# ydwu4/dgl-hack

Measured on AMD Instinct MI355X. Metric: edges/sec + achieved HBM GB/s, GCN copy_u_sum on 100M-edge graph, 1/2/4/8 MI355X, higher is better.
Workload: dtype f32; 1 GPU; M1 copy_u_sum: RMAT scale 23, 100000000 edges, feat 64, int32 in-CSR; nodes=8388608, edges=100000000, feat=64, parallelism=single

## Files before the change

dgl-hack_amd/csrc/capi.cpp:

```cpp
#include <hip/hip_runtime.h>

#include <algorithm>
#include <cmath>
#include <atomic>
#include <cstdio>
#include <cstdlib>
#include <cstring>
#include <stdexcept>
#include <string>
#include <vector>

#include "internal.h"

using namespace dglmi;

namespace {

thread_local std::string g_last_error;

struct Error : std::runtime_error {
  using std::runtime_error::runtime_error;
};

#define DGLMI_CHECK(cond, msg)                                                     \
// ... 308 lines not shown
    prev = dst;
  }
}

void run_fast(const ReduceWalk& rw, int kind, int red, const float* x, const int32_t* x_map,
              const float* w, const int32_t* w_map, float* out, int64_t F, int64_t head_dim,
              hipStream_t s, const DGLMIEpilogue* epi, const float* xr) {
  const DGLMICsr& walk = rw.csr;
  if (rw.num_blocks > 1 && !rw.wide && red == RED_SUM && x_map == nullptr && walk.nnz > 0 &&
      kind == FAST_COPY_COL && rw.blocks != nullptr) {
    run_fast_blocked(rw, kind, x, w, w_map, out, F, head_dim, s, epi);
    return;
  }
  if (walk.nnz == 0) {
    launch_fill(out, walk.num_rows * F, identity_of(red), s);
    if (epi) launch_epilogue(out, walk.num_rows, F, epi->row_mul, epi->row_div, epi->bias, epi->addend, s);
    return;
  }
  FastArgs a;
  std::memset(&a, 0, sizeof(a));
  a.indptr = rw.idx(walk.indptr);
  a.rows = walk.rows;
  a.indices = walk.indices;
  a.eids = rw.idx(rw.eid_positions ? nullptr : walk.data);
  a.nnz = walk.nnz;
  a.num_rows = walk.num_rows;
  a.x = x;
  a.w = w;
  a.x_map = x_map;
  a.w_map = w_map;
  a.out = out;
  a.F = F;
  a.head_dim = head_dim;
  a.chunk = fast_chunk_edges(walk.nnz, F);
  a.xr = xr;
  if (kind == FAST_COPY_COL && red == RED_SUM && x_map == nullptr && fast_marked_supported(F) &&
      rw.marked != nullptr &&
      walk.num_cols * F * static_cast<int64_t>(sizeof(float)) >= kMarkedMinTableBytes) {
    a.indices = rw.marked;
    a.marked = 1;
    a.num_cols = walk.num_cols;
  }
  if (epi) {
    a.row_mul = epi->row_mul;
    a.row_div = epi->row_div;
    a.bias = epi->bias;
    a.addend = epi->addend;
  }
  if (kind == FAST_COL_MUL_EDGE_BCAST && !a.eids && head_dim == F && w_map == nullptr &&
      red == RED_SUM)
    kind = FAST_COL_MUL_POS;
  const DGLMIHubPlan* plan = rw.plan;
  if (plan != nullptr && !(kind == FAST_COPY_COL && red == RED_SUM && x_map == nullptr && epi == nullptr &&
                           !rw.wide && fast_marked_supported(F) && plan->num_hubs > 0))
    plan = nullptr;
  const int64_t virt = plan ? plan->num_blocks * plan->num_hubs : 0;
  Scratch part(no_workspace(), virt * F * static_cast<int64_t>(sizeof(float)), s);
  if (plan != nullptr) {
    DGLMI_CHECK(plan->nnz == walk.nnz && plan->hub_nnz <= walk.nnz && plan->num_blocks >= 1 &&
                    plan->rows && plan->indices && plan->indptr && plan->hub_rows,
                "hub plan does not belong to this CSR");
    a.indptr = IdxPtr{plan->indptr, 0};
    a.rows = plan->rows;
    a.indices = plan->marked ? plan->marked : plan->indices;
    a.marked = plan->marked != nullptr;
    a.num_cols = walk.num_cols;
    a.num_rows = virt + walk.num_rows;
    a.part = static_cast<float*>(part.ptr);
    a.virt_rows = virt;
    a.hub_rows = plan->hub_rows;
    a.num_hubs = plan->num_hubs;
    a.hub_blocks = plan->num_blocks;
    a.hub_nnz = plan->hub_nnz;
  }
  const CarryLayout lay((walk.nnz + a.chunk - 1) / a.chunk, F);
  Scratch carry(rw.ws, lay.bytes, s);
  lay.point(a, carry.ptr);
  launch_fast_reduce(kind, red, a, s);
  check_hip(hipGetLastError(), "fast reduce launch");
}

std::atomic<int> g_sddmm_order{DGLMI_SDDMM_ORDER_AUTO};

SddmmArgs sddmm_items(const DGLMIGraph* g, const DGLMICsr& walk, bool edge_operand,
                      int64_t row_floats) {
  SddmmArgs e;
  std::memset(&e, 0, sizeof(e));
  e.nnz = walk.nnz;
  bool coo = g->coo_src != nullptr && g->coo_dst != nullptr;
  if (coo) {
    const int forced = g_sddmm_order.load(std::memory_order_relaxed);
    if (forced == DGLMI_SDDMM_ORDER_CSR) coo = false;
    else if (forced != DGLMI_SDDMM_ORDER_COO)
      coo = edge_operand || row_floats < 32 || walk.nnz < 64 * std::max<int64_t>(walk.num_rows, 1);
  }
  if (coo) {
    e.rows = g->coo_dst;
    e.cols = g->coo_src;
    e.eids = IdxPtr{nullptr, 0};
  } else {
    e.rows = walk.rows;
    e.cols = walk.indices;
    e.eids = idx(g, walk.data);
  }
  return e;
}

EdgeArgs base_args(const DGLMIGraph* g, const DGLMICsr& walk) {
  EdgeArgs a;
  std::memset(&a, 0, sizeof(a));
  a.indptr = idx(g, walk.indptr);
  a.indices = walk.indices;
  a.eids = idx(g, walk.data);
  a.rows = walk.rows;
  a.num_rows = walk.num_rows;
  a.nnz = walk.nnz;
  a.len = 1;
  return a;
}

struct ReduceShape {
  bool bc;
  Bcast binfo;
  int64_t D, len;
};

// ... 1976 lines not shown
```

dgl-hack_amd/csrc/internal.h:

```cpp
#pragma once

#include <hip/hip_runtime.h>

#include <cstdint>

#include "../../include/dglmi.h"

namespace dglmi {

enum Role : int { ROLE_ROW = 0, ROLE_COL = 1, ROLE_EDGE = 2, ROLE_NONE = 3 };
enum Red : int { RED_SUM = 0, RED_MAX = 1, RED_MIN = 2, RED_PROD = 3, RED_NONE = 4 };
enum Op : int { OP_ADD = 0, OP_SUB = 1, OP_MUL = 2, OP_DIV = 3, OP_DOT = 4, OP_USE_LHS = 5 };

constexpr int kMaxDim = DGLMI_MAX_NDIM;

struct IdxPtr {
  const void* p;
  int wide;
  __host__ __device__ __forceinline__ int64_t operator[](int64_t i) const {
    return wide ? static_cast<const int64_t*>(p)[i]
                : static_cast<int64_t>(static_cast<const int32_t*>(p)[i]);
  }
  __host__ __device__ __forceinline__ explicit operator bool() const { return p != nullptr; }
};
// ... 240 lines not shown
  int pack;
  float* stat_pk;
};
bool softmax_supported(int64_t H);

bool project_supported(int64_t K, int64_t N);
int project_instance(int64_t K, int64_t N);
void launch_project(const float* X, int64_t M, int64_t K, const float* W, int64_t swk, int64_t swn,
                    int64_t N, const float* bias, float* Y, hipStream_t s);
int64_t softmax_chunk_edges(int64_t nnz, int64_t H);
int64_t softmax_owned_carry_bytes(int64_t nnz, int64_t H);
void launch_edge_softmax(const SoftmaxArgs& a, bool backward, hipStream_t s);
void launch_sm_row_sums(const SoftmaxArgs& a, hipStream_t s);

enum FastKind : int {
  FAST_COPY_COL = 0,
  FAST_COPY_EDGE = 1,
  FAST_COL_MUL_EDGE = 2,
  FAST_COL_MUL_EDGE_BCAST = 3,
  FAST_COL_TIE = 4,
  FAST_COL_MUL_POS = 5,
};
struct FastArgs {
  IdxPtr indptr;
  const int32_t* rows;
  const int32_t* indices;
  IdxPtr eids;
  int64_t nnz;
  int64_t num_rows;
  const float* x;
  const float* w;
  const int32_t* x_map;
  const int32_t* w_map;
  float* out;
  int64_t F;
  int64_t head_dim;
  float* carry;
  int32_t* seg_cnt;
  int64_t chunk;
  const float* row_mul;
  const float* row_div;
  const float* bias;
  const float* addend;
  int marked;
  const float* xr;
  int64_t num_cols;
  float* part;
  int64_t virt_rows;
  const int32_t* hub_rows;
  int64_t num_hubs;
  int64_t hub_blocks;
  int64_t hub_nnz;
  int64_t plan_wgs;
};
int64_t fast_chunk_edges(int64_t nnz, int64_t F);
int64_t fast_workspace_bytes(int64_t nnz, int64_t F);
bool fast_supported(int kind, int64_t F, int64_t head_dim);
void launch_fast_reduce(int kind, int red, const FastArgs& a, hipStream_t s);
void launch_mark_cold(const int32_t* cols, int64_t nnz, IdxPtr deg_indptr, int32_t thresh,
                      int32_t* out_cols, hipStream_t s);
inline bool fast_marked_supported(int64_t F) { return F > 32 && F <= 256 && F % 4 == 0; }
constexpr int64_t kMarkedMinTableBytes = int64_t(256) << 20;

struct GatArgs {
  const int32_t* indptr;
  const int32_t* rows;
  const int32_t* indices;
  int64_t nnz;
  int64_t num_rows;
  int H, D;
  int64_t F;
  float slope;
  const float* ft;
  const float* el;
  const float* er;
  float* out;
  float* m;
  float* l;
  const float* go;
  const float* fo;
  const float* m_in;
  const float* l_in;
  float4* stats;
  float* g_er;
  float* g_el;
  float* g_ft;
  float* carry;
  int32_t* seg_cnt;
  int64_t chunk;
  int raw;
  int accumulate;
  int skip_stats;
  int o32;
  float* t;
  int64_t t_off;
  float* lf;
  float* ls;
  int drop;
  uint32_t drop_thresh;
  float drop_scale;
  uint64_t drop_seed;
  const void* drop_bits;
  int drop_width;
  int drop_pos;
  int64_t drop_off;
  int drop_rng;
  int rng_vec;
  int rng_shift;
  float rng_keep;
  uint64_t rng_seed;
  uint64_t rng_ctr;
  int64_t rng_threads;
  const int32_t* eids;
// ... 126 lines not shown
```

dgl-hack_amd/csrc/spmm_chunk.h:

```cpp
#pragma once
#include "internal.h"

#include <climits>
#include <cstdlib>

namespace dglmi {
namespace {

constexpr int kBlock = 256;

template <int VW> struct VecT;
template <> struct VecT<4> { using T = float4; };
template <> struct VecT<2> { using T = float2; };
template <> struct VecT<1> { using T = float; };

__device__ __forceinline__ float4 ld4(const float* p) {
  return *reinterpret_cast<const float4*>(p);
}
__device__ __forceinline__ void st4(float* p, float4 v) { *reinterpret_cast<float4*>(p) = v; }
typedef float f32x4 __attribute__((ext_vector_type(4)));
typedef float f32x2 __attribute__((ext_vector_type(2)));

template <int VW>
__device__ __forceinline__ typename VecT<VW>::T vld(const float* p) {
  return *reinterpret_cast<const typename VecT<VW>::T*>(p);
}
template <int VW>
__device__ __forceinline__ typename VecT<VW>::T vld_nt(const float* p) {
  if constexpr (VW == 4) {
    const f32x4 v = __builtin_nontemporal_load(reinterpret_cast<const f32x4*>(p));
    return make_float4(v.x, v.y, v.z, v.w);
  } else if constexpr (VW == 2) {
    const f32x2 v = __builtin_nontemporal_load(reinterpret_cast<const f32x2*>(p));
    return make_float2(v.x, v.y);
  } else {
    return __builtin_nontemporal_load(p);
  }
}
__device__ __forceinline__ void vst(float* p, float4 v) { st4(p, v); }
__device__ __forceinline__ void vst(float* p, float2 v) { *reinterpret_cast<float2*>(p) = v; }
__device__ __forceinline__ void vst(float* p, float v) { *p = v; }
__device__ __forceinline__ void vst_nt(float* p, float4 v) {
  __builtin_nontemporal_store(v.x, p);
  __builtin_nontemporal_store(v.y, p + 1);
  __builtin_nontemporal_store(v.z, p + 2);
  __builtin_nontemporal_store(v.w, p + 3);
}
__device__ __forceinline__ void vst_nt(float* p, float2 v) {
  __builtin_nontemporal_store(v.x, p);
  __builtin_nontemporal_store(v.y, p + 1);
}
__device__ __forceinline__ void vst_nt(float* p, float v) { __builtin_nontemporal_store(v, p); }

template <int RED>
__device__ __forceinline__ float4 vred(float4 a, float4 b) {
  return make_float4(red_apply<RED>(a.x, b.x), red_apply<RED>(a.y, b.y),
                     red_apply<RED>(a.z, b.z), red_apply<RED>(a.w, b.w));
// ... 73 lines not shown
  } else if constexpr (KIND == FAST_COL_MUL_POS) {
    const int64_t c = a.x_map ? a.x_map[col] : col;
    return vld<VW>(a.x + c * a.F + VW * fv);
  } else {
    const int64_t c = a.x_map ? a.x_map[col] : col;
    const int64_t e = a.w_map ? a.w_map[eid] : eid;
    return vscale(vld<VW>(a.x + c * a.F + VW * fv), a.w[e * wn + hs]);
  }
}

template <int VAR>
__device__ __forceinline__ int32_t ld_stream(const int32_t* p) {
  if constexpr (VAR & 1) return __builtin_nontemporal_load(p);
  else return *p;
}
template <int VAR>
__device__ __forceinline__ int64_t ld_stream(IdxPtr q, int64_t p) {
  if (q.wide) {
    const int64_t* x = static_cast<const int64_t*>(q.p) + p;
    if constexpr (VAR & 1) return __builtin_nontemporal_load(x);
    else return *x;
  }
  return ld_stream<VAR>(static_cast<const int32_t*>(q.p) + p);
}
template <int VAR>
__device__ __forceinline__ float ld_stream_f(const float* p) {
  if constexpr (VAR & 1) return __builtin_nontemporal_load(p);
  else return *p;
}
template <int VAR, typename V>
__device__ __forceinline__ void st_out(float* p, V v) {
  if constexpr (VAR & 2) vst_nt(p, v);
  else vst(p, v);
}

template <bool EPI, int VW>
__device__ __forceinline__ typename VecT<VW>::T epiv(const FastArgs& a, typename VecT<VW>::T v,
                                                    int64_t r, int fv) {
  if constexpr (EPI) {
    if (a.row_mul) v = vscale(v, a.row_mul[r]);
    if (a.row_div) v = vdivs(v, a.row_div[r]);
    if (a.bias) v = vadd(v, vld<VW>(a.bias + VW * fv));
    if (a.addend) v = vadd(v, vld<VW>(a.addend + r * a.F + VW * fv));
  }
  return v;
}

template <bool PLAN>
__device__ __forceinline__ float* row_dst(const FastArgs& a, int64_t r) {
  if constexpr (PLAN) return r < a.virt_rows ? a.part + r * a.F : a.out + (r - a.virt_rows) * a.F;
  else return a.out + r * a.F;
}

template <int KIND, int RED, int L, int NV, int VAR = 3, bool EPI = false, int VW = 4, bool PLAN = false>
__global__ void __launch_bounds__(kBlock) k_chunk_reduce(FastArgs a, IdxPtr indptr) {
  static_assert(!PLAN || !EPI, "the plan variant has no epilogue");
  static_assert(L >= 1 && L <= 64, "a lane group must fit in one wavefront (fill_empty_rows)");
  constexpr int G = kBlock / L;
  constexpr int B = (L > 16 ? L : 16) * ((VAR & 4) ? 2 : 1);
  constexpr int U = (NV == 1 ? 8 : (NV == 2 ? 4 : 2)) * ((VAR & 4) ? 2 : 1);
  static_assert(B % U == 0, "B must be a multiple of U");
  __shared__ int32_t s_row[G][B];
  __shared__ int32_t s_col[G][B];
  __shared__ int64_t s_eid[needs_eid<KIND>() ? G : 1][needs_eid<KIND>() ? B : 1];
  constexpr bool kScalarW = KIND == FAST_COL_MUL_POS;
  __shared__ float s_w[kScalarW ? G : 1][kScalarW ? B : 1];

  const int g = threadIdx.x / L;
  const int lane = threadIdx.x % L;
  int64_t bid = blockIdx.x;
  if constexpr (PLAN) {
    if (bid < a.plan_wgs) bid = (bid % 8) * (a.plan_wgs / 8) + bid / 8;
  }
  const int64_t chunk = bid * G + g;
  const int64_t K = a.chunk;
  const int64_t p0 = chunk * K;
  if (p0 >= a.nnz) return;
  const int64_t p1 = p0 + K < a.nnz ? p0 + K : a.nnz;
  seg_reset(a.seg_cnt, chunk, lane);
  using V = typename VecT<VW>::T;
  const int F4 = static_cast<int>(a.F / VW);
  const V I = vident<VW, RED>();
  [[maybe_unused]] const __amdgpu_buffer_rsrc_t rsrc =
      __builtin_amdgcn_make_buffer_rsrc(const_cast<float*>(a.x), 0, -1, 0x00020000);
  int hsel[NV];
  const int64_t wn = KIND == FAST_COL_MUL_EDGE_BCAST ? a.F / a.head_dim : 1;
#pragma unroll
  for (int v = 0; v < NV; ++v)
    hsel[v] = KIND == FAST_COL_MUL_EDGE_BCAST ? static_cast<int>((VW * (lane + v * L)) / a.head_dim) : 0;

  int64_t cur = a.rows[p0];
  bool cont = p0 > 0 && a.rows[p0 - 1] == cur;
  V acc[NV];
#pragma unroll
  for (int v = 0; v < NV; ++v) acc[v] = I;

  constexpr int SQ = B / L;
  constexpr bool kEid = needs_eid<KIND>();
  int32_t nr[SQ], nc[SQ];
  [[maybe_unused]] int64_t ne[kEid ? SQ : 1];
  [[maybe_unused]] float nw[kScalarW ? SQ : 1];
  auto fetch = [&](int64_t nb) {
#pragma unroll
    for (int i = 0; i < SQ; ++i) {
      const int64_t p = nb + lane + i * L;
      const bool ok = p < p1;
      nr[i] = ok ? ld_stream<VAR>(a.rows + p) : INT_MAX;
      nc[i] = ok ? ld_stream<VAR>(a.indices + p) : 0;
      if constexpr (kEid) ne[kEid ? i : 0] = ok ? (a.eids ? ld_stream<VAR>(a.eids, p) : p) : 0;
      if constexpr (kScalarW) nw[kScalarW ? i : 0] = ok ? ld_stream_f<VAR>(a.w + p) : 0.0f;
    }
  };
  fetch(p0);
  for (int64_t base = p0; base < p1; base += B) {
#pragma unroll
    for (int i = 0; i < SQ; ++i) {
      const int q = lane + i * L;
      s_row[g][q] = nr[i];
      s_col[g][q] = nc[i];
      if constexpr (kEid) s_eid[kEid ? g : 0][q] = ne[kEid ? i : 0];
      if constexpr (kScalarW) s_w[kScalarW ? g : 0][kScalarW ? q : 0] = nw[kScalarW ? i : 0];
    }
    __builtin_amdgcn_fence(__ATOMIC_RELEASE, "wavefront");
    __builtin_amdgcn_wave_barrier();
    __builtin_amdgcn_fence(__ATOMIC_ACQUIRE, "wavefront");
    if (base + B < p1) fetch(base + B);
    constexpr bool kMulVec = KIND == FAST_COL_MUL_EDGE;
    constexpr bool kMulScl = KIND == FAST_COL_MUL_EDGE_BCAST || KIND == FAST_COL_MUL_POS;
    constexpr bool kTie = KIND == FAST_COL_TIE;
    constexpr bool kTwo = kMulVec || kTie;
#pragma unroll
    for (int ub = 0; ub < B; ub += U) {
      V val[U][NV];
      [[maybe_unused]] V wv[kTwo ? U : 1][kTwo ? NV : 1];
      [[maybe_unused]] float wsc[kMulScl ? U : 1][kMulScl ? NV : 1];
      bool fast_mul = false;
      if constexpr (kMulVec || kMulScl || kTie) fast_mul = a.x_map == nullptr && a.w_map == nullptr;
      if (fast_mul) {
        if constexpr (kMulVec || kMulScl || kTie) {
        int64_t cc[U], ee[U];
        bool okk[U];
#pragma unroll
        for (int u = 0; u < U; ++u) {
          cc[u] = s_col[g][ub + u];
          okk[u] = s_row[g][ub + u] != INT_MAX;
          if constexpr (!kScalarW && !kTie) ee[u] = s_eid[needs_eid<KIND>() ? g : 0][ub + u];
        }
#pragma unroll
        for (int u = 0; u < U; ++u)
#pragma unroll
          for (int v = 0; v < NV; ++v) {
            const int f4 = lane + v * L;
            val[u][v] = (okk[u] && f4 < F4) ? vld<VW>(a.x + cc[u] * a.F + VW * f4) : I;
          }
#pragma unroll
        for (int u = 0; u < U; ++u)
#pragma unroll
          for (int v = 0; v < NV; ++v) {
            const int f4 = lane + v * L;
            const bool in = okk[u] && f4 < F4;
            if constexpr (kScalarW)
              wsc[u][kMulScl ? v : 0] = s_w[kScalarW ? g : 0][kScalarW ? ub + u : 0];
            else if constexpr (kMulScl)
              wsc[u][kMulScl ? v : 0] = in ? a.w[ee[u] * wn + hsel[v]] : 0.0f;
            else if constexpr (kTie)
              wv[kTwo ? u : 0][kTwo ? v : 0] = in ? vld<VW>(a.w + cc[u] * a.F + VW * f4) : I;
            else
              wv[kTwo ? u : 0][kTwo ? v : 0] = in ? vld<VW>(a.w + ee[u] * a.F + VW * f4) : I;
          }
        }
      } else {
#pragma unroll
      for (int u = 0; u < U; ++u) {
        const int32_t col = s_col[g][ub + u];
        const int64_t eid = needs_eid<KIND>() ? s_eid[needs_eid<KIND>() ? g : 0][ub + u] : 0;
        const bool ok = s_row[g][ub + u] != INT_MAX;
#pragma unroll
        for (int v = 0; v < NV; ++v) {
          const int f4 = lane + v * L;
          if constexpr ((VAR & kVarBuf) != 0 && KIND == FAST_COPY_COL && VW == 4) {
            const bool cold = col < 0;
            const uint32_t off = (static_cast<uint32_t>(col & 0x7fffffff) * static_cast<uint32_t>(a.F) +
                                  static_cast<uint32_t>(VW * f4)) * 4u;
            if (ok && f4 < F4)
              val[u][v] = cold ? buf_ld4<(VAR >> 5) & 31>(rsrc, off) : buf_ld4<(VAR >> 10) & 31>(rsrc, off);
            else
              val[u][v] = I;
          } else if constexpr ((VAR & 8) != 0 && KIND == FAST_COPY_COL) {
            const bool nt = (col < 0) != ((VAR & 16) != 0);
            const float* px = a.x + static_cast<int64_t>(col & 0x7fffffff) * a.F + VW * f4;
            val[u][v] = (ok && f4 < F4) ? (nt ? vld_nt<VW>(px) : vld<VW>(px)) : I;
          } else {
            val[u][v] = (ok && f4 < F4) ? edge_value<KIND, VW>(a, col, eid, f4, hsel[v], wn, s_row[g][ub + u]) : I;
            if constexpr (kScalarW) wsc[u][kMulScl ? v : 0] = s_w[kScalarW ? g : 0][kScalarW ? ub + u : 0];
            else if constexpr (kMulScl) wsc[u][kMulScl ? v : 0] = 1.0f;
            if constexpr (kMulVec) wv[kTwo ? u : 0][kTwo ? v : 0] = vone<VW>();
          }
        }
      }
      }
#pragma unroll
      for (int u = 0; u < U; ++u) {
        const int32_t r = s_row[g][ub + u];
        if (r == INT_MAX) break;
        if (r != cur) {
          float* dst = cont ? a.carry + chunk * a.F : row_dst<PLAN>(a, cur);
#pragma unroll
          for (int v = 0; v < NV; ++v) {
            const int f4 = lane + v * L;
            if (f4 < F4) st_out<VAR>(dst + VW * f4, cont ? acc[v] : epiv<EPI, VW>(a, acc[v], cur, f4));
            acc[v] = I;
          }
          cur = r;
          cont = false;
        }
#pragma unroll
        for (int v = 0; v < NV; ++v) {
          if constexpr (kMulVec) acc[v] = vred<RED>(acc[v], vmul(val[u][v], wv[kTwo ? u : 0][kTwo ? v : 0]));
          else if constexpr (kTie) {
            const int f4 = lane + v * L;
            acc[v] = vred<RED>(acc[v], fast_mul && f4 < F4
                                           ? vtie(vld<VW>(a.xr + static_cast<int64_t>(r) * a.F + VW * f4),
                                                  wv[kTwo ? u : 0][kTwo ? v : 0], val[u][v])
                                           : val[u][v]);
          }
          else if constexpr (kMulScl) acc[v] = vred<RED>(acc[v], vscale(val[u][v], wsc[u][kMulScl ? v : 0]));
          else acc[v] = vred<RED>(acc[v], val[u][v]);
        }
      }
    }
    __builtin_amdgcn_wave_barrier();
  }
  {
    float* dst = cont ? a.carry + chunk * a.F : row_dst<PLAN>(a, cur);
    const bool done = !cont && !(EPI && p1 < a.nnz && a.rows[p1] == cur);
#pragma unroll
    for (int v = 0; v < NV; ++v) {
      const int f4 = lane + v * L;
      if (f4 < F4) st_out<VAR>(dst + VW * f4, done ? epiv<EPI, VW>(a, acc[v], cur, f4) : acc[v]);
    }
  }
  fill_empty_rows(indptr, a.num_rows, chunk, (a.nnz + K - 1) / K, L, lane, [&](int64_t r) {
#pragma unroll
    for (int v = 0; v < NV; ++v) {
      const int f4 = lane + v * L;
      if (f4 < F4) st_out<VAR>(row_dst<PLAN>(a, r) + VW * f4, epiv<EPI, VW>(a, I, r, f4));
    }
  });
}

template <int RED, int L, int NV, bool EPI = false, int VW = 4, bool PLAN = false>
__global__ void __launch_bounds__(kBlock) k_chunk_fixup(FastArgs a, IdxPtr indptr) {
  static_assert(L >= 1 && L <= 64, "a lane group must fit in one wavefront (seg_arrive_last)");
  constexpr int G = kBlock / L;
  const int lane = threadIdx.x % L;
  const FixupRole w = fixup_role(a, indptr, (int64_t)blockIdx.x * G + threadIdx.x / L);
  if (!w.work) return;
  using V = typename VecT<VW>::T;
// ... 213 lines not shown
```

dgl-hack_amd/dgl/_ffi.py:

```python
from __future__ import annotations

import ctypes
import os

MAX_NDIM = 8


class DGLError(Exception):
    """Error raised by the engine (python/dgl/_ffi/base.py:24)."""


class CSR(ctypes.Structure):
    _fields_ = [
        ("num_rows", ctypes.c_int64),
        ("num_cols", ctypes.c_int64),
        ("nnz", ctypes.c_int64),
        ("indptr", ctypes.c_void_p),
        ("indices", ctypes.c_void_p),
        ("data", ctypes.c_void_p),
        ("rows", ctypes.c_void_p),
    ]


class Graph(ctypes.Structure):
    _fields_ = [
        ("in_csr", CSR),
        ("out_csr", CSR),
        ("num_bits", ctypes.c_int32),
        ("device", ctypes.c_int32),
        ("workspace", ctypes.c_void_p),
        ("workspace_bytes", ctypes.c_int64),
        ("coo_src", ctypes.c_void_p),
        ("coo_dst", ctypes.c_void_p),
        ("in_gather_cols", ctypes.c_void_p),
        ("out_gather_cols", ctypes.c_void_p),
        ("num_col_blocks", ctypes.c_int32),
        ("in_col_blocks", ctypes.c_void_p),
        ("out_col_blocks", ctypes.c_void_p),
        ("rgcn", ctypes.c_void_p),
        ("gat_edge_pos", ctypes.c_void_p),
        ("etypes", ctypes.c_void_p),
        ("eid_identity", ctypes.c_int32),
        ("in_hub_plan", ctypes.c_void_p),
        ("out_hub_plan", ctypes.c_void_p),
    ]


class HubPlan(ctypes.Structure):
    _fields_ = [
        ("num_blocks", ctypes.c_int32),
        ("num_hubs", ctypes.c_int64),
        ("hub_nnz", ctypes.c_int64),
        ("nnz", ctypes.c_int64),
        ("rows", ctypes.c_void_p),
        ("indices", ctypes.c_void_p),
        ("marked", ctypes.c_void_p),
        ("indptr", ctypes.c_void_p),
        ("hub_rows", ctypes.c_void_p),
    ]


class RgcnState(ctypes.Structure):
    _fields_ = [
        ("etypes", ctypes.c_void_p),
        ("norm", ctypes.c_void_p),
        ("num_rels", ctypes.c_int32),
        ("layers", ctypes.c_int32),
        ("num_src", ctypes.c_int64),
        ("nnz", ctypes.c_int64),
        ("positions", ctypes.c_void_p),
        ("in_cols", ctypes.c_void_p * 2),
        ("in_norm", ctypes.c_void_p),
        ("out_typed", CSR * 2),
        ("out_norm", ctypes.c_void_p * 2),
        ("in_rel", CSR),
        ("in_rel_norm", ctypes.c_void_p),
        ("owner", ctypes.c_void_p),
    ]


class Epilogue(ctypes.Structure):
    _fields_ = [
        ("row_mul", ctypes.c_void_p),
        ("row_div", ctypes.c_void_p),
        ("bias", ctypes.c_void_p),
        ("addend", ctypes.c_void_p),
    ]


class DropoutDraw(ctypes.Structure):
    _fields_ = [
        ("seed", ctypes.c_uint64),
        ("offset", ctypes.c_uint64),
        ("threads", ctypes.c_int64),
        ("vec", ctypes.c_int32),
        ("keep", ctypes.c_float),
        ("scale", ctypes.c_float),
    ]


class Array(ctypes.Structure):
    _fields_ = [
        ("data", ctypes.c_void_p),
        ("ndim", ctypes.c_int32),
        ("shape", ctypes.c_int64 * (MAX_NDIM + 1)),
    ]


def _lib_name():
    return "libdglmi_probes.so" if os.environ.get("DGLMI_PROBES") == "1" else "libdglmi.so"

# ... 261 lines not shown
```

dgl-hack_amd/dgl/graph_index.py:

```python
from __future__ import annotations

import ctypes
import os

import weakref

import numpy as np
import torch as th

from . import _ffi
from ._ffi import DGLError


def _ptr(t):
    return ctypes.c_void_p(t.data_ptr()) if t is not None else None


class DeviceCSR:

    def __init__(self, indptr, indices, data, rows, num_cols):
        self.bits = 64 if indptr.dtype == th.int64 else 32
        self.indptr = indptr
        self.indices = indices
        self.data = data
        self.rows = rows
        self.num_rows = int(indptr.shape[0]) - 1
        self.num_cols = int(num_cols)
        self.nnz = int(indices.shape[0])

    def cstruct(self):
        if getattr(self, "_c", None) is None:
            self._c = self._make_cstruct()
        return _ffi.CSR.from_buffer_copy(self._c)

    def _make_cstruct(self):
        c = _ffi.CSR()
        c.num_rows = self.num_rows
        c.num_cols = self.num_cols
        c.nnz = self.nnz
        c.indptr = self.indptr.data_ptr()
        c.indices = self.indices.data_ptr() if self.nnz else None
        c.data = self.data.data_ptr() if self.nnz else None
        c.rows = self.rows.data_ptr() if self.nnz else None
        return c

    def degrees(self):
        if getattr(self, "_deg", None) is None:
            self._deg = self.indptr[1:] - self.indptr[:-1]
        return self._deg


def build_hub_plan(indptr, indices, rows, hub_degree, nb=8):
    num_rows = int(indptr.shape[0]) - 1
    is_hub = (indptr[1:] - indptr[:-1]) >= hub_degree
    hub_rows = th.nonzero(is_hub).reshape(-1)
    nh = int(hub_rows.shape[0])
    if nh == 0:
        return None
    rank = th.cumsum(is_hub.long(), 0) - 1
    pos_hub = is_hub[rows.long()]
    hub_pos = th.nonzero(pos_hub).reshape(-1)
    light_pos = th.nonzero(~pos_hub).reshape(-1)
    del pos_hub
    hcols = indices[hub_pos].long()
    n_he = int(hcols.shape[0])
    cuts = th.sort(hcols).values[[(k * n_he) // nb for k in range(1, nb)]]
    block = th.bucketize(hcols, cuts.contiguous(), right=True)
    vrow = block * nh + rank[rows[hub_pos].long()]
    del hcols, block
    order = th.argsort(vrow, stable=True)
    virt = nb * nh
    positions = th.cat([hub_pos[order], light_pos])
    plan_rows = th.cat([vrow[order], rows[light_pos].long() + virt])
    del order, vrow, hub_pos, light_pos
    out_ptr = th.zeros(virt + num_rows + 1, dtype=th.int64, device=indptr.device)
    out_ptr[1:] = th.cumsum(th.bincount(plan_rows, minlength=virt + num_rows), 0)
    return {"num_blocks": nb, "num_hubs": nh, "hub_nnz": n_he, "positions": positions,
            "rows": plan_rows.to(th.int32), "indices": indices[positions].contiguous(),
            "indptr": out_ptr.to(th.int32), "hub_rows": hub_rows.to(th.int32),
            "cuts": cuts}


class ImmutableGraphIndex:

    def __init__(self, in_csr, out_csr, num_src, num_dst, device, eid_perm=False):
        self.in_csr = in_csr
        self.out_csr = out_csr
        self.num_src = num_src
        self.num_dst = num_dst
        self.device = device
        self.eid_perm = eid_perm
        self._coo = None
        self._gather_cols = None
        self._col_blocks = {}
        self.position_of = None
        self.etypes = None

    def set_edge_types(self, etypes):
        if etypes is None:
            self.etypes = None
            return self
        t = th.as_tensor(etypes).reshape(-1)
        if t.numel() != self.in_csr.nnz:
            raise DGLError("etypes needs one entry per edge (%d, got %d)"
                           % (self.in_csr.nnz, t.numel()))
        if t.numel() and int(t.min()) < 0:
            raise DGLError("negative edge type")
        self.etypes = t.to(device=self.in_csr.indices.device, dtype=th.int32).contiguous()
        return self

    def number_of_edges(self):
        return self.in_csr.nnz

    @property
    def num_bits(self):
        return self.in_csr.bits

    def coo(self):
        if not self.eid_perm:
            return None
        if self._coo is None:
            c = self.in_csr
            src = th.empty(c.nnz, dtype=th.int32, device=c.indices.device)
            dst = th.empty_like(src)
            if c.nnz:
                e = c.data.long()
                src[e] = c.indices
                dst[e] = c.rows
            self._coo = (src, dst)
        return self._coo

    HOT_DEGREE = 64
    MAX_COLD_SHARE = 0.5
# ... 13 lines not shown
                        continue
                    out = th.empty(csr.nnz, dtype=th.int32, device=csr.indices.device)
                    _ffi.check_call(_ffi.lib().DGLMIKernelMarkColdColumns(
                        ctypes.byref(g), direction, hot, out.data_ptr(),
                        th.cuda.current_stream(csr.indices.device).cuda_stream))
                    if float((out < 0).float().mean()) > self.MAX_COLD_SHARE:
                        out = None
                    cols.append(out)
                self._gather_cols = tuple(cols)
        return self._gather_cols

    HUB_DEGREE = 128
    HUB_BLOCKS = 8
    HUB_HOT_DEGREE = 8
    HUB_MIN_TABLE_BYTES = 256 << 20
    HUB_MIN_EDGE_SHARE = 0.25
    HUB_MAX_PARTIAL_SHARE = 0.10

    def hub_plan(self, direction, feat_len):
        csr = self.in_csr if direction == "in" else self.out_csr
        if (csr.bits != 32 or not (32 < feat_len <= 256 and feat_len % 4 == 0)
                or csr.num_cols * feat_len * 4 < self.HUB_MIN_TABLE_BYTES):
            return None
        plans = self.__dict__.setdefault("_hub_plans", {})
        if direction not in plans:
            plans[direction] = self._make_hub_plan(direction, csr)
        return plans[direction]

    def _make_hub_plan(self, direction, csr):
        deg = int(os.environ.get("DGLMI_HUB_DEGREE", self.HUB_DEGREE))
        if deg <= 0 or csr.nnz == 0:
            return None
        p = build_hub_plan(csr.indptr, csr.indices, csr.rows, deg, self.HUB_BLOCKS)
        if p is None:
            return None
        virt = p["num_blocks"] * p["num_hubs"]
        if (p["hub_nnz"] < self.HUB_MIN_EDGE_SHARE * csr.nnz
                or 2 * virt > self.HUB_MAX_PARTIAL_SHARE * csr.nnz
                or virt + csr.num_rows >= MAX_NODES):
            return None
        hints = self.gather_cols()[0 if direction == "in" else 1]
        marked = None
        if hints is not None:
            marked = hints[p["positions"]]
            hot = os.environ.get("DGLMI_HUB_HOT_DEGREE", self.HUB_HOT_DEGREE)
            if hot is not None:
                h = p["hub_nnz"]
                cols = p["indices"][:h]
                count = th.bincount(csr.indices.long(), minlength=csr.num_cols)
                marked[:h] = th.where(count[cols.long()] < int(hot), cols | (-2 ** 31), cols)
        c = _ffi.HubPlan()
        c.num_blocks, c.num_hubs = p["num_blocks"], p["num_hubs"]
        c.hub_nnz, c.nnz = p["hub_nnz"], csr.nnz
        keep = (p["rows"], p["indices"], marked, p["indptr"], p["hub_rows"])
        c.rows, c.indices = keep[0].data_ptr(), keep[1].data_ptr()
        c.marked = marked.data_ptr() if marked is not None else None
        c.indptr, c.hub_rows = keep[3].data_ptr(), keep[4].data_ptr()
        c._keep = keep
        return c

    @staticmethod
    def _split_by_column(csr, nb):
        dev = csr.indices.device
        n_rows = csr.num_rows
        key = (csr.indices.long() * nb) // max(1, csr.num_cols)
        order = th.argsort(key, stable=True)
        counts = th.bincount(key, minlength=nb).tolist()
        rows, cols, data = csr.rows[order], csr.indices[order], csr.data[order]
        del order, key
        out, start = [], 0
        for b in range(nb):
            end = start + counts[b]
            r = rows[start:end]
            indptr = th.zeros(n_rows + 1, dtype=th.int64, device=dev)
            indptr[1:] = th.cumsum(th.bincount(r.long(), minlength=n_rows), 0)
            out.append(DeviceCSR(indptr.to(th.int32), cols[start:end], data[start:end], r,
                                 csr.num_cols))
            start = end
        return out

    def position_operand(self, w, direction="in"):
        ic, oc = self.in_csr, self.out_csr
        view = self.position_view(direction)
        walk = ic if direction == "in" else oc
        key = self._operand_key(w)
        owner = w._base if w._base is not None else w
        cached = self._pos_operands.get(direction)
        if cached is None or cached[0] != key or cached[1]() is not owner:
            ops = self._pos_operands

            def drop(ref, direction=direction):
                ent = ops.get(direction)
                if ent is not None and ent[1] is ref:
                    del ops[direction]
            from . import kernel as K
            cached = (key, weakref.ref(owner, drop), K.gather_rows(w, walk.data))
            self._pos_operands[direction] = cached
        return view, cached[2]

    def clear_operand_cache(self):
        if getattr(self, "_pos_operands", None) is not None:
            self._pos_operands.clear()
        self._operand_seen = None

    @staticmethod
    def _operand_key(w):
        return (w.data_ptr(), w._version, tuple(w.shape), tuple(w.stride()), w.dtype)

    def reused_operand(self, w):
        key = self._operand_key(w)
# ... 434 lines not shown
```

include/dglmi.h:

```cpp
#ifndef DGLMI_H_
#define DGLMI_H_

#include <stdint.h>

#ifdef __cplusplus
extern "C" {
#endif

#define DGLMI_MAX_NDIM 8

enum DGLMITarget {
  DGLMI_TARGET_SRC = 0,
  DGLMI_TARGET_DST = 1,
  DGLMI_TARGET_EDGE = 2,
  DGLMI_TARGET_NONE = 3
};

typedef struct {
  int64_t num_rows;
  int64_t num_cols;
  int64_t nnz;
  const int32_t* indptr;
  const int32_t* indices;
  const int32_t* data;
  const int32_t* rows;
} DGLMICsr;

typedef struct {
  DGLMICsr in_csr;
  DGLMICsr out_csr;
  int32_t num_bits;
  int32_t device;
  void* workspace;
  int64_t workspace_bytes;
  const int32_t* coo_src;
  const int32_t* coo_dst;
  const int32_t* in_gather_cols;
  const int32_t* out_gather_cols;
  int32_t num_col_blocks;
  const DGLMICsr* in_col_blocks;
  const DGLMICsr* out_col_blocks;
  const struct DGLMIRgcnState* rgcn;
  const int32_t* gat_edge_pos;
  const int32_t* etypes;
  int32_t eid_identity;
  const struct DGLMIHubPlan* in_hub_plan;
  const struct DGLMIHubPlan* out_hub_plan;
} DGLMIGraph;

typedef struct DGLMIHubPlan {
  int32_t num_blocks;
  int64_t num_hubs;
  int64_t hub_nnz;
  int64_t nnz;
  const int32_t* rows;
  const int32_t* indices;
  const int32_t* marked;
  const int32_t* indptr;
  const int32_t* hub_rows;
} DGLMIHubPlan;

typedef struct {
  float* data;
  int32_t ndim;
  int64_t shape[DGLMI_MAX_NDIM + 1];
} DGLMIArray;

typedef struct {
  const float* row_mul;
  const float* row_div;
  const float* bias;
  const float* addend;
} DGLMIEpilogue;

const char* DGLMIGetLastError(void);

const char* DGLMIVersion(void);

enum DGLMISddmmOrder {
  DGLMI_SDDMM_ORDER_AUTO = 0,
  DGLMI_SDDMM_ORDER_COO = 1,
  DGLMI_SDDMM_ORDER_CSR = 2
};
int DGLMISetSddmmOrder(int32_t order);

int DGLMIKernelInferBinaryFeatureShape(const char* op, const DGLMIArray* lhs,
                                       const DGLMIArray* rhs, int64_t* out_shape,
                                       int32_t* out_ndim);

int DGLMIKernelBinaryOpReduce(const char* reducer, const char* op, const DGLMIGraph* graph,
                              int32_t lhs_target, int32_t rhs_target,
                              const DGLMIArray* lhs, const DGLMIArray* rhs, DGLMIArray* out,
                              const int32_t* lhs_mapping, const int32_t* rhs_mapping,
                              const int32_t* out_mapping, void* stream);

int DGLMIKernelBackwardLhsBinaryOpReduce(
    const char* reducer, const char* op, const DGLMIGraph* graph, int32_t lhs_target,
    int32_t rhs_target, const int32_t* lhs_mapping, const int32_t* rhs_mapping,
    const int32_t* out_mapping, const DGLMIArray* lhs, const DGLMIArray* rhs,
    const DGLMIArray* out, const DGLMIArray* grad_out, DGLMIArray* grad_lhs, void* stream);

int DGLMIKernelBackwardRhsBinaryOpReduce(
    const char* reducer, const char* op, const DGLMIGraph* graph, int32_t lhs_target,
    int32_t rhs_target, const int32_t* lhs_mapping, const int32_t* rhs_mapping,
    const int32_t* out_mapping, const DGLMIArray* lhs, const DGLMIArray* rhs,
    const DGLMIArray* out, const DGLMIArray* grad_out, DGLMIArray* grad_rhs, void* stream);

int DGLMIKernelCopyReduce(const char* reducer, const DGLMIGraph* graph, int32_t target,
                          const DGLMIArray* in, DGLMIArray* out, const int32_t* in_mapping,
                          const int32_t* out_mapping, void* stream);

int DGLMIKernelBinaryOpReduceEx(const char* reducer, const char* op, const DGLMIGraph* graph,
// ... 226 lines not shown
```

Before: 36.89 billion edges/s.

## Replace per-edge row array with row-start bitmap in hub-plan SpMM walk

In the hub-plan copy_u_sum kernel, the per-edge int32 row stream is replaced by a bitmap of row starts (one bit per edge), a per-word prefix rank, and a compact list of distinct row ids. Each wavefront loads a bitmap word per lane, uses popcounts to find segment boundaries and looks up the row id only when flushing. This cuts index traffic from 8 to about 4 bytes per edge plus row ids per segment. It costs extra host-side preprocessing and popcount/shared-memory work. The plan is now limited to chunks of at most 512 edges.

```diff
diff --git a/dgl-hack_amd/csrc/capi.cpp b/dgl-hack_amd/csrc/capi.cpp
--- a/dgl-hack_amd/csrc/capi.cpp
+++ b/dgl-hack_amd/csrc/capi.cpp
@@ -384,13 +384,15 @@
     kind = FAST_COL_MUL_POS;
   const DGLMIHubPlan* plan = rw.plan;
   if (plan != nullptr && !(kind == FAST_COPY_COL && red == RED_SUM && x_map == nullptr && epi == nullptr &&
-                           !rw.wide && fast_marked_supported(F) && plan->num_hubs > 0))
+                           !rw.wide && fast_marked_supported(F) && plan->num_hubs > 0 &&
+                           a.chunk <= kPlanMaxChunk))
     plan = nullptr;
   const int64_t virt = plan ? plan->num_blocks * plan->num_hubs : 0;
   Scratch part(no_workspace(), virt * F * static_cast<int64_t>(sizeof(float)), s);
   if (plan != nullptr) {
     DGLMI_CHECK(plan->nnz == walk.nnz && plan->hub_nnz <= walk.nnz && plan->num_blocks >= 1 &&
-                    plan->rows && plan->indices && plan->indptr && plan->hub_rows,
+                    plan->rows && plan->indices && plan->indptr && plan->hub_rows &&
+                    plan->starts && plan->start_rank && plan->row_ids,
                 "hub plan does not belong to this CSR");
     a.indptr = IdxPtr{plan->indptr, 0};
     a.rows = plan->rows;
@@ -404,6 +406,9 @@
     a.num_hubs = plan->num_hubs;
     a.hub_blocks = plan->num_blocks;
     a.hub_nnz = plan->hub_nnz;
+    a.starts = plan->starts;
+    a.start_rank = plan->start_rank;
+    a.row_ids = plan->row_ids;
   }
   const CarryLayout lay((walk.nnz + a.chunk - 1) / a.chunk, F);
   Scratch carry(rw.ws, lay.bytes, s);
diff --git a/dgl-hack_amd/csrc/internal.h b/dgl-hack_amd/csrc/internal.h
--- a/dgl-hack_amd/csrc/internal.h
+++ b/dgl-hack_amd/csrc/internal.h
@@ -316,6 +316,9 @@
   int64_t hub_blocks;
   int64_t hub_nnz;
   int64_t plan_wgs;
+  const uint32_t* starts;
+  const int32_t* start_rank;
+  const int32_t* row_ids;
 };
 int64_t fast_chunk_edges(int64_t nnz, int64_t F);
 int64_t fast_workspace_bytes(int64_t nnz, int64_t F);
@@ -323,6 +326,7 @@
 void launch_fast_reduce(int kind, int red, const FastArgs& a, hipStream_t s);
 void launch_mark_cold(const int32_t* cols, int64_t nnz, IdxPtr deg_indptr, int32_t thresh,
                       int32_t* out_cols, hipStream_t s);
+constexpr int64_t kPlanMaxChunk = 32 * 16;
 inline bool fast_marked_supported(int64_t F) { return F > 32 && F <= 256 && F % 4 == 0; }
 constexpr int64_t kMarkedMinTableBytes = int64_t(256) << 20;
 
diff --git a/dgl-hack_amd/csrc/spmm_chunk.h b/dgl-hack_amd/csrc/spmm_chunk.h
--- a/dgl-hack_amd/csrc/spmm_chunk.h
+++ b/dgl-hack_amd/csrc/spmm_chunk.h
@@ -3,6 +3,7 @@
 
 #include <climits>
 #include <cstdlib>
+#include <type_traits>
 
 namespace dglmi {
 namespace {
@@ -182,6 +183,9 @@
   else return a.out + r * a.F;
 }
 
+__device__ __forceinline__ int popcount_bits(uint32_t v) { return __popc(v); }
+__device__ __forceinline__ int popcount_bits(uint64_t v) { return __popcll(v); }
+
 template <int KIND, int RED, int L, int NV, int VAR = 3, bool EPI = false, int VW = 4, bool PLAN = false>
 __global__ void __launch_bounds__(kBlock) k_chunk_reduce(FastArgs a, IdxPtr indptr) {
   static_assert(!PLAN || !EPI, "the plan variant has no epilogue");
@@ -190,7 +194,10 @@
   constexpr int B = (L > 16 ? L : 16) * ((VAR & 4) ? 2 : 1);
   constexpr int U = (NV == 1 ? 8 : (NV == 2 ? 4 : 2)) * ((VAR & 4) ? 2 : 1);
   static_assert(B % U == 0, "B must be a multiple of U");
-  __shared__ int32_t s_row[G][B];
+  static_assert(!PLAN || (B == L && KIND == FAST_COPY_COL), "the plan walk: one position and one window entry per lane");
+  __shared__ int32_t s_row[PLAN ? 1 : G][PLAN ? 1 : B];
+  __shared__ uint32_t s_bits[PLAN ? G : 1][PLAN ? L : 1];
+  __shared__ int32_t s_win[PLAN ? G : 1][PLAN ? B : 1];
   __shared__ int32_t s_col[G][B];
   __shared__ int64_t s_eid[needs_eid<KIND>() ? G : 1][needs_eid<KIND>() ? B : 1];
   constexpr bool kScalarW = KIND == FAST_COL_MUL_POS;
@@ -227,26 +234,66 @@
 
   constexpr int SQ = B / L;
   constexpr bool kEid = needs_eid<KIND>();
-  int32_t nr[SQ], nc[SQ];
+  [[maybe_unused]] int32_t nr[SQ];
+  int32_t nc[SQ];
   [[maybe_unused]] int64_t ne[kEid ? SQ : 1];
   [[maybe_unused]] float nw[kScalarW ? SQ : 1];
-  auto fetch = [&](int64_t nb) {
-#pragma unroll
-    for (int i = 0; i < SQ; ++i) {
-      const int64_t p = nb + lane + i * L;
-      const bool ok = p < p1;
-      nr[i] = ok ? ld_stream<VAR>(a.rows + p) : INT_MAX;
-      nc[i] = ok ? ld_stream<VAR>(a.indices + p) : 0;
-      if constexpr (kEid) ne[kEid ? i : 0] = ok ? (a.eids ? ld_stream<VAR>(a.eids, p) : p) : 0;
-      if constexpr (kScalarW) nw[kScalarW ? i : 0] = ok ? ld_stream_f<VAR>(a.w + p) : 0.0f;
+  using Bits = std::conditional_t<(B > 32), uint64_t, uint32_t>;
+  [[maybe_unused]] Bits bits = 0;
+  [[maybe_unused]] int64_t win0 = 0;
+  [[maybe_unused]] int32_t nwin = 0;
+  [[maybe_unused]] const int sh = static_cast<int>(p0 & 31);
+  [[maybe_unused]] auto batch_bits = [&](int64_t nb) -> Bits {
+    const int o = static_cast<int>(nb - p0) + sh;
+    const int n = p1 - nb < B ? static_cast<int>(p1 - nb) : B;
+    if constexpr (B > 32) {
+      const uint64_t v = ((static_cast<uint64_t>(s_bits[PLAN ? g : 0][PLAN ? (o >> 5) + 1 : 0]) << 32) |
+                          s_bits[PLAN ? g : 0][PLAN ? o >> 5 : 0]) >> (o & 31);
+      return n >= 64 ? v : v & ((uint64_t(1) << n) - 1);
+    } else {
+      const uint32_t v = s_bits[PLAN ? g : 0][PLAN ? o >> 5 : 0] >> (o & 31);
+      return n >= 32 ? v : v & ((1u << n) - 1u);
     }
   };
-  fetch(p0);
+  auto fetch = [&](int64_t nb, [[maybe_unused]] bool cols = true) {
+    if constexpr (PLAN) {
+      if (cols) nc[0] = nb + lane < p1 ? ld_stream<VAR>(a.indices + nb + lane) : 0;
+      win0 += popcount_bits(bits);
+      bits = batch_bits(nb);
+      if (nb == p0) bits &= ~Bits(1);
+      nwin = lane < popcount_bits(bits) ? a.row_ids[win0 + lane] : 0;
+    } else {
+#pragma unroll
+      for (int i = 0; i < SQ; ++i) {
+        const int64_t p = nb + lane + i * L;
+        const bool ok = p < p1;
+        nr[i] = ok ? ld_stream<VAR>(a.rows + p) : INT_MAX;
+        nc[i] = ok ? ld_stream<VAR>(a.indices + p) : 0;
+        if constexpr (kEid) ne[kEid ? i : 0] = ok ? (a.eids ? ld_stream<VAR>(a.eids, p) : p) : 0;
+        if constexpr (kScalarW) nw[kScalarW ? i : 0] = ok ? ld_stream_f<VAR>(a.w + p) : 0.0f;
+      }
+    }
+  };
+  if constexpr (PLAN) {
+    const int64_t w0 = p0 >> 5;
+    const uint32_t word = (w0 + lane) * 32 < p1 ? a.starts[w0 + lane] : 0u;
+    const int32_t rank0 = a.start_rank[w0];
+    nc[0] = p0 + lane < p1 ? ld_stream<VAR>(a.indices + p0 + lane) : 0;
+    s_bits[PLAN ? g : 0][PLAN ? lane : 0] = word;
+    __builtin_amdgcn_fence(__ATOMIC_RELEASE, "wavefront");
+    __builtin_amdgcn_wave_barrier();
+    __builtin_amdgcn_fence(__ATOMIC_ACQUIRE, "wavefront");
+    win0 = rank0 + __popc(s_bits[PLAN ? g : 0][0] & ((2u << sh) - 1u));
+    fetch(p0, false);
+  } else {
+    fetch(p0);
+  }
   for (int64_t base = p0; base < p1; base += B) {
 #pragma unroll
     for (int i = 0; i < SQ; ++i) {
       const int q = lane + i * L;
-      s_row[g][q] = nr[i];
+      if constexpr (PLAN) s_win[PLAN ? g : 0][PLAN ? q : 0] = nwin;
+      else s_row[PLAN ? 0 : g][PLAN ? 0 : q] = nr[i];
       s_col[g][q] = nc[i];
       if constexpr (kEid) s_eid[kEid ? g : 0][q] = ne[kEid ? i : 0];
       if constexpr (kScalarW) s_w[kScalarW ? g : 0][kScalarW ? q : 0] = nw[kScalarW ? i : 0];
@@ -254,6 +301,8 @@
     __builtin_amdgcn_fence(__ATOMIC_RELEASE, "wavefront");
     __builtin_amdgcn_wave_barrier();
     __builtin_amdgcn_fence(__ATOMIC_ACQUIRE, "wavefront");
+    [[maybe_unused]] const Bits cb = bits;
+    [[maybe_unused]] const int cn = p1 - base < B ? static_cast<int>(p1 - base) : B;
     if (base + B < p1) fetch(base + B);
     constexpr bool kMulVec = KIND == FAST_COL_MUL_EDGE;
     constexpr bool kMulScl = KIND == FAST_COL_MUL_EDGE_BCAST || KIND == FAST_COL_MUL_POS;
@@ -304,7 +353,9 @@
       for (int u = 0; u < U; ++u) {
         const int32_t col = s_col[g][ub + u];
         const int64_t eid = needs_eid<KIND>() ? s_eid[needs_eid<KIND>() ? g : 0][ub + u] : 0;
-        const bool ok = s_row[g][ub + u] != INT_MAX;
+        [[maybe_unused]] int32_t srow = 0;
+        if constexpr (!PLAN) srow = s_row[PLAN ? 0 : g][PLAN ? 0 : ub + u];
+        const bool ok = PLAN ? ub + u < cn : srow != INT_MAX;
 #pragma unroll
         for (int v = 0; v < NV; ++v) {
           const int f4 = lane + v * L;
@@ -321,7 +372,7 @@
             const float* px = a.x + static_cast<int64_t>(col & 0x7fffffff) * a.F + VW * f4;
             val[u][v] = (ok && f4 < F4) ? (nt ? vld_nt<VW>(px) : vld<VW>(px)) : I;
           } else {
-            val[u][v] = (ok && f4 < F4) ? edge_value<KIND, VW>(a, col, eid, f4, hsel[v], wn, s_row[g][ub + u]) : I;
+            val[u][v] = (ok && f4 < F4) ? edge_value<KIND, VW>(a, col, eid, f4, hsel[v], wn, srow) : I;
             if constexpr (kScalarW) wsc[u][kMulScl ? v : 0] = s_w[kScalarW ? g : 0][kScalarW ? ub + u : 0];
             else if constexpr (kMulScl) wsc[u][kMulScl ? v : 0] = 1.0f;
             if constexpr (kMulVec) wv[kTwo ? u : 0][kTwo ? v : 0] = vone<VW>();
@@ -331,9 +382,18 @@
       }
 #pragma unroll
       for (int u = 0; u < U; ++u) {
-        const int32_t r = s_row[g][ub + u];
-        if (r == INT_MAX) break;
-        if (r != cur) {
+        int32_t r = 0;
+        bool flush;
+        if constexpr (PLAN) {
+          if (ub + u >= cn) break;
+          flush = (cb >> (ub + u)) & 1;
+        } else {
+          r = s_row[PLAN ? 0 : g][PLAN ? 0 : ub + u];
+          if (r == INT_MAX) break;
+          flush = r != cur;
+        }
+        if (flush) {
+          if constexpr (PLAN) r = s_win[PLAN ? g : 0][PLAN ? popcount_bits(cb & ((Bits(1) << (ub + u)) - 1)) : 0];
           float* dst = cont ? a.carry + chunk * a.F : row_dst<PLAN>(a, cur);
 #pragma unroll
           for (int v = 0; v < NV; ++v) {
diff --git a/dgl-hack_amd/dgl/_ffi.py b/dgl-hack_amd/dgl/_ffi.py
--- a/dgl-hack_amd/dgl/_ffi.py
+++ b/dgl-hack_amd/dgl/_ffi.py
@@ -57,6 +57,9 @@
         ("marked", ctypes.c_void_p),
         ("indptr", ctypes.c_void_p),
         ("hub_rows", ctypes.c_void_p),
+        ("starts", ctypes.c_void_p),
+        ("start_rank", ctypes.c_void_p),
+        ("row_ids", ctypes.c_void_p),
     ]
 
 
diff --git a/dgl-hack_amd/dgl/graph_index.py b/dgl-hack_amd/dgl/graph_index.py
--- a/dgl-hack_amd/dgl/graph_index.py
+++ b/dgl-hack_amd/dgl/graph_index.py
@@ -75,10 +75,27 @@
     del order, vrow, hub_pos, light_pos
     out_ptr = th.zeros(virt + num_rows + 1, dtype=th.int64, device=indptr.device)
     out_ptr[1:] = th.cumsum(th.bincount(plan_rows, minlength=virt + num_rows), 0)
-    return {"num_blocks": nb, "num_hubs": nh, "hub_nnz": n_he, "positions": positions,
+    plan = {"num_blocks": nb, "num_hubs": nh, "hub_nnz": n_he, "positions": positions,
             "rows": plan_rows.to(th.int32), "indices": indices[positions].contiguous(),
             "indptr": out_ptr.to(th.int32), "hub_rows": hub_rows.to(th.int32),
             "cuts": cuts}
+    plan.update(plan_row_starts(plan["rows"]))
+    return plan
+
+
+def plan_row_starts(rows):
+    nnz = int(rows.shape[0])
+    first = th.ones(nnz, dtype=th.bool, device=rows.device)
+    first[1:] = rows[1:] != rows[:-1]
+    at = th.nonzero(first).reshape(-1)
+    del first
+    words = (nnz + 31) // 32 + 1
+    bits = th.zeros(words, dtype=th.int64, device=rows.device)
+    bits.index_add_(0, at >> 5, th.ones_like(at) << (at & 31))
+    count = th.bincount(at >> 5, minlength=words)
+    return {"starts": th.where(bits >= 2 ** 31, bits - 2 ** 32, bits).to(th.int32),
+            "start_rank": (th.cumsum(count, 0) - count).to(th.int32),
+            "row_ids": rows[at].to(th.int32).contiguous()}
 
 
 class ImmutableGraphIndex:
@@ -198,10 +215,12 @@
         c = _ffi.HubPlan()
         c.num_blocks, c.num_hubs = p["num_blocks"], p["num_hubs"]
         c.hub_nnz, c.nnz = p["hub_nnz"], csr.nnz
-        keep = (p["rows"], p["indices"], marked, p["indptr"], p["hub_rows"])
+        keep = (p["rows"], p["indices"], marked, p["indptr"], p["hub_rows"],
+                p["starts"], p["start_rank"], p["row_ids"])
         c.rows, c.indices = keep[0].data_ptr(), keep[1].data_ptr()
         c.marked = marked.data_ptr() if marked is not None else None
         c.indptr, c.hub_rows = keep[3].data_ptr(), keep[4].data_ptr()
+        c.starts, c.start_rank, c.row_ids = (t.data_ptr() for t in keep[5:])
         c._keep = keep
         return c
 
diff --git a/include/dglmi.h b/include/dglmi.h
--- a/include/dglmi.h
+++ b/include/dglmi.h
@@ -58,6 +58,9 @@
   const int32_t* marked;
   const int32_t* indptr;
   const int32_t* hub_rows;
+  const uint32_t* starts;
+  const int32_t* start_rank;
+  const int32_t* row_ids;
 } DGLMIHubPlan;
 
 typedef struct {
```

New measurement: 37.88 billion edges/s (median of 6 runs). +2.7%, better.
